# tigert1998/ray-tracing-cuda

Hardware: AMD Instinct MI355X
Metric: Mrays/s (higher is better)
Workload: dtype f32

## Files before the change

ray-tracing-cuda_amd/csrc/capi.hip:

```cpp
#include <hip/hip_runtime.h>
#include <dlfcn.h>
#include <rccl/rccl.h>
#include <string.h>

#include <algorithm>
#include <cmath>
#include <cstdlib>
#include <mutex>
#include <string>
#include <unordered_map>

#include "../../include/rtmi.h"
#include "kernels.h"
#include "scene.h"
#include "xorwow.h"

using namespace rtmi;

static thread_local std::string g_err;
static int fail(int code, const std::string &msg) {
  g_err = msg;
  return code;
}
static int hip_fail(hipError_t e, const char *what) {
  return fail(RTMI_ERR_HIP, std::string(what) + ": " + hipGetErrorString(e));
}
#define HIP_TRY(expr)                                    \
  do {                                                   \
    hipError_t e__ = (expr);                             \
    if (e__ != hipSuccess) return hip_fail(e__, #expr);  \
  } while (0)

// ... 383 lines not shown
  free_device(s);
  std::string err = s->flatten();
  if (!err.empty()) return fail(RTMI_ERR_INVALID, err);
  HIP_TRY(hipGetDevice(&s->device));
  s->tex_recs.clear();
  for (const HostTex &t : s->texs) {
    if (!t.image) continue;
    void *d = nullptr;
    size_t pitch = 0;
    HIP_TRY(hipMallocPitch(&d, &pitch, (size_t)t.w * 4, (size_t)t.h));
    s->dev_allocs.push_back(d);
    HIP_TRY(hipMemcpy2D(d, pitch, t.rgba.data(), (size_t)t.w * 4, (size_t)t.w * 4, (size_t)t.h,
                        hipMemcpyHostToDevice));
    TexRec r{};
    r.rgba = reinterpret_cast<const uint8_t *>(d);
    r.height = t.h, r.width = t.w, r.pitch = (int64_t)pitch;
    s->tex_recs.push_back(r);
  }
  SceneDev d{};
  int rc;
  if ((rc = upload(s, s->runs, &d.runs))) return rc;
  if ((rc = upload(s, s->spheres, &d.spheres))) return rc;
  if ((rc = upload(s, s->tris, &d.tris))) return rc;
  if ((rc = upload(s, s->pair_boxes, &d.pair_boxes))) return rc;
  if ((int)s->pair_pts.size() <= kLdsPairs && (rc = upload(s, s->tri_pts, &d.tri_pts))) return rc;
  if ((rc = upload(s, s->tri_nrm, &d.tri_nrm))) return rc;
  if ((rc = upload(s, s->sph_groups, &d.sph_groups))) return rc;
  if ((rc = upload(s, s->sph_members, &d.sph_members))) return rc;
  d.sph_mag = s->sph_mag;
  d.n_sph_groups = (int)s->sph_groups.size();
  if ((rc = upload(s, s->bvh_recs, &d.bvhs))) return rc;
  if ((rc = upload(s, s->nodes, &d.nodes))) return rc;
  if ((rc = upload(s, s->qnodes, &d.qnodes))) return rc;
  if ((rc = upload(s, s->leaf_paths, &d.leaf_paths))) return rc;
  if ((rc = upload(s, s->tops, &d.tops))) return rc;
  if ((rc = upload(s, s->faces, &d.faces))) return rc;
  if ((rc = upload(s, s->face_uv, &d.face_uv))) return rc;
#ifdef RTMI_CHECK_MARGINS
  if ((rc = upload(s, s->face_of_orig, &d.face_of_orig))) return rc;
#endif
  if ((rc = upload(s, s->mat_recs, &d.mats))) return rc;
  if ((rc = upload(s, s->tex_recs, &d.texs))) return rc;
  d.n_runs = (int)s->runs.size() - 4;
  d.n_pairs = (int)s->pair_pts.size();
  d.list_mag = s->list_mag;
  d.n_mats = (int)s->mat_recs.size();
  d.n_nodes = (int)s->nodes.size();
// ... 59 lines not shown
  Scene tmp;
  if (int rc = flattened(sp, &tmp)) return rc;
  return tmp.sliver_faces;
}

int64_t rtmi_scene_bytes_per_ray(const rtmi_scene *sp) {
  if (!sp) return fail(RTMI_ERR_INVALID, "null scene");
  Scene tmp;
  if (int rc = flattened(sp, &tmp)) return rc;
  return tmp.bytes_per_ray;
}

int64_t rtmi_debug_list_records(const rtmi_scene *sp, int64_t cap_pairs, uint32_t *tri_pts, uint32_t *hot_tris, float *corners) {
  if (!sp) return fail(RTMI_ERR_INVALID, "null scene");
  Scene tmp;
  if (int rc = flattened(sp, &tmp)) return rc;
  const int64_t n = (int64_t)tmp.pair_pts.size();
  for (int64_t i = 0; i < n && i < cap_pairs; i++) {
    if (tri_pts) memcpy(tri_pts + 24 * i, &tmp.tri_pts[2 * i], 2 * sizeof(TriPts));
    if (hot_tris) memcpy(hot_tris + 32 * i, &tmp.tris[2 * i], 2 * sizeof(HotTri));
    if (corners) memcpy(corners + 12 * i, tmp.pair_pts[i].p0, 12 * sizeof(float));
  }
  return n;
}

int64_t rtmi_debug_render_lds_bytes(const rtmi_scene *sp, int max_depth, int threads) {
  if (!sp || max_depth < 0 || threads < 64 || threads % 64) return fail(RTMI_ERR_INVALID, "bad arguments");
  Scene tmp;
  if (int rc = flattened(sp, &tmp)) return rc;
  SceneDev d{};
  d.n_pairs = (int)tmp.pair_pts.size(), d.n_mats = (int)tmp.mat_recs.size(), d.n_nodes = (int)tmp.nodes.size();
  d.n_leaf_paths = (int)tmp.leaf_paths.size(), d.n_sph_groups = (int)tmp.sph_groups.size();
  FrameDev fr{};
  fr.max_depth = max_depth;
  return (int64_t)render_lds_bytes(pick_variant(tmp.features), d, fr, threads);
}

int64_t rtmi_frame_work_items(const rtmi_frame *f) {
  FrameDev d;
  if (!make_frame(f, &d)) return fail(RTMI_ERR_INVALID, frame_why("bad frame"));
  return d.items;
}
int64_t rtmi_frame_pixel_of(const rtmi_frame *f, int64_t q) {
  FrameDev d;
  if (!make_frame(f, &d) || q < 0 || q >= d.items) return -1;
  return frame_pixel_of(d, d.rank, q);
// ... 867 lines not shown
```

ray-tracing-cuda_amd/csrc/closest_hit.h:

```cpp
#pragma once

#ifdef RTMI_CHECK_MARGINS
__device__ inline bool aabb_hit_reference(const BvhNode &nd, V3 o, V3 d, double t_from, double t_to) {
  const float oo[3] = {o.x, o.y, o.z}, dd[3] = {d.x, d.y, d.z};
  for (int i = 0; i < 3; i++) {
    if (dd[i] == 0.f) continue;
    for (int s = 0; s < 2; s++) {
      const float tf = ((s == 0 ? nd.mn[i] : nd.mx[i]) - oo[i]) / dd[i];
      const double t = (double)tf;
      if (t != t || fabs(t) == (double)INFINITY) continue;
      if (!(t_from <= t && t <= t_to)) continue;
      const float pt[3] = {oo[0] + (float)t * dd[0], oo[1] + (float)t * dd[1], oo[2] + (float)t * dd[2]};
      bool inside = true;
      for (int a = 0; a < 3; a++)
        if (a != i && !(nd.mn[a] <= pt[a] && pt[a] <= nd.mx[a])) inside = false;
      if (inside) return true;
    }
  }
  return false;
}
template <typename T>
__device__ inline bool bvh_reference_walk(const SceneDev &sc, const BvhRec &br, V3 o, V3 d, T &t_to, int &face, float &fu,
                                          float &fv) {
  int stk_node[kRefDepthMax + 2], stk_first[kRefDepthMax + 2], stk_n[kRefDepthMax + 2];
// ... 53 lines not shown
                                           , double t_start = INFINITY, double t_stop = INFINITY, bool *uncertain = nullptr
) {
  constexpr bool DT = (F & F_SPHERE) != 0;
  typedef typename TSel<DT>::type T;
  bool ok = false;
  T t_to = OCC ? (T)t_start : (T)INFINITY;
#define RTMI_DECIDED (OCC && ok && t_to <= (T)t_stop)
  uint32_t win = ID_NONE;
  int32_t aux = 0;
  int32_t work = 0;
  float bu = 0.f, bv = 0.f;

  double sa = 0.0, sa2 = 0.0;
  float saf = 0.f;
  if (F & F_SPHERE) {
    float la = len3(d);
    saf = la * la;
    sa = (double)saf;
    sa2 = 2 * sa;
  }

  const int lane = (int)(threadIdx.x & 63u);
  const bool det_safe = (M & PIN_DET_SAFE) || sc.det_safe != 0;
  const bool cull_list = (F & F_TRIS) && ((M & PIN_LDS_TABLES) || (ll != nullptr && sc.n_pairs >= kCullMinPairs));
  V3 cull_inv = splat(0.f), cull_klo = splat(0.f), cull_khi = splat(0.f);
  if ((F & F_TRIS) && cull_list) {
    const float ix = __builtin_amdgcn_rcpf(d.x), iy = __builtin_amdgcn_rcpf(d.y), iz = __builtin_amdgcn_rcpf(d.z);
    cull_inv = mk(fabsf(d.x) < 1e-30f ? copysignf(1e30f, d.x) : ix, fabsf(d.y) < 1e-30f ? copysignf(1e30f, d.y) : iy,
                  fabsf(d.z) < 1e-30f ? copysignf(1e30f, d.z) : iz);
    const float delta = MESH_DIST_SLACK * (fmaxf(fmaxf(fabsf(o.x), fabsf(o.y)), fabsf(o.z)) + sc.list_mag);
    cull_klo = mk(-(o.x + delta) * cull_inv.x, -(o.y + delta) * cull_inv.y, -(o.z + delta) * cull_inv.z);
    cull_khi = mk(-(o.x - delta) * cull_inv.x, -(o.y - delta) * cull_inv.y, -(o.z - delta) * cull_inv.z);
  }

  for (int ri = 0; ri < sc.n_runs; ri++) {
    if (OCC) {
      live = live && !RTMI_DECIDED;
      if (__builtin_amdgcn_ballot_w64(live) == 0ull) break;
    }
    const i32x4 rv = load_run(sc.runs, ri);
    Run run;
    run.kind = rv[0], run.first = rv[1], run.count = rv[2], run.pad = rv[3];
    if (live && run.kind == RUN_SKY) {
      const T ts = (T)1e9f;
      bool hit = ts <= t_to;
      bool acc = hit && (!ok || ts < t_to);
      ok = ok || acc;
      t_to = acc ? ts : t_to;
      win = acc ? make_id(RUN_SKY, 0) : win;
    }
    if ((F & F_TRIS) && run.kind == RUN_TRIS && cull_list) {
      const int pair0 = run.first >> 1;
      const float lo0 = T_FROM_F * kTimeLo;
      for (int c0 = 0; c0 < run.count; c0 += 32) {
        if (OCC && __builtin_amdgcn_ballot_w64(live && !RTMI_DECIDED) == 0ull) break;
        const int nc = run.count - c0 < 32 ? run.count - c0 : 32;
        const float hi0 = (float)t_to * kTimeHi + kTimeAbs;
        uint32_t mask = 0u;
        RTMI_STAT2(const unsigned long long tc0 = stat_now();)
#define RTMI_CULL_PAIR(bx)                                                                                                      \
  {                                                                                                                             \
    const float t0x = __builtin_fmaf(bx[0], cull_inv.x, cull_klo.x), t1x = __builtin_fmaf(bx[3], cull_inv.x, cull_khi.x); \
    const float t0y = __builtin_fmaf(bx[1], cull_inv.y, cull_klo.y), t1y = __builtin_fmaf(bx[4], cull_inv.y, cull_khi.y); \
    const float t0z = __builtin_fmaf(bx[2], cull_inv.z, cull_klo.z), t1z = __builtin_fmaf(bx[5], cull_inv.z, cull_khi.z); \
    const float en = fmaxf(fmaxf(fminf(t0x, t1x), fminf(t0y, t1y)), fminf(t0z, t1z));                                            \
    const float le = fminf(fminf(fmaxf(t0x, t1x), fmaxf(t0y, t1y)), fmaxf(t0z, t1z));                                            \
    cull_step(mask, fmaxf(lo0, en), fminf(hi0, le));                                                                            \
  }
        f32x8 A = load_pair_box(sc.pair_boxes, pair0 + c0), B;
        int i = 0;
        for (; i + 1 < nc; i += 2) {
          __builtin_amdgcn_s_waitcnt(0xc07f);
          __builtin_amdgcn_sched_barrier(0);
          B = load_pair_box(sc.pair_boxes, pair0 + c0 + i + 1);
          __builtin_amdgcn_sched_barrier(0);
          RTMI_CULL_PAIR(A)
          __builtin_amdgcn_s_waitcnt(0xc07f);
          __builtin_amdgcn_sched_barrier(0);
          A = load_pair_box(sc.pair_boxes, pair0 + c0 + i + 2);
          __builtin_amdgcn_sched_barrier(0);
          RTMI_CULL_PAIR(B)
        }
        if (i < nc) {
          __builtin_amdgcn_s_waitcnt(0xc07f);
          __builtin_amdgcn_sched_barrier(0);
          RTMI_CULL_PAIR(A)
        }
#undef RTMI_CULL_PAIR
        mask = __brev(mask) >> (32 - nc);
        if (!live) mask = 0u;
        if (OCC && RTMI_DECIDED) mask = 0u;
        RTMI_STAT2(const unsigned long long tc1 = stat_now(); st.cyc[5] += tc1 - tc0;)
        RTMI_STAT(st.cull_bits += (unsigned)__popcll(__builtin_amdgcn_ballot_w64(true)) * 0u; { unsigned pc = __builtin_popcount(mask); for (int off = 32; off > 0; off >>= 1) pc += __shfl_down(pc, off); st.cull_bits += __builtin_amdgcn_readfirstlane(pc); } st.cull_rays += (unsigned)__popcll(__builtin_amdgcn_ballot_w64(true));)
#ifndef RTMI_OWN_FIRST
#define RTMI_OWN_FIRST 1
#endif
#if RTMI_OWN_FIRST
        if (__builtin_amdgcn_ballot_w64(mask != 0u) != 0ull) {
          if (mask != 0u) {
            const int bit = __builtin_ctz(mask);
            mask &= mask - 1u;
            const int rec = 2 * (pair0 + c0 + bit);
            V3 p0, e1, e2, p1, e1b, e2b;
            (void)load_tri_pts<M>(sc, s_tris, rec, 0, p0, e1, e2);
            const bool second = load_tri_pts<M>(sc, s_tris, rec + 1, 1, p1, e1b, e2b);
            float ta = 0.f, ua = 0.f, va = 0.f, tb = 0.f, ub = 0.f, vb = 0.f;
            const bool hit_a = tri_test_flat<T>(p0, e1, e2, cross3(d, e2), o, d, t_to, ta, ua, va, det_safe);
            bool hit_b = false;
            if (second) hit_b = tri_test_flat<T>(p1, e1b, e2b, cross3(d, e2b), o, d, t_to, tb, ub, vb, det_safe) && !hit_a;
            const float t = hit_a ? ta : tb;
// ... 580 lines not shown
```

ray-tracing-cuda_amd/csrc/kernels.h:

```cpp
#pragma once
#include <hip/hip_runtime.h>
#include <stdint.h>

#include "../../include/rtmi.h"
#include "scene_dev.h"

#define RTMI_KERNEL_MAX_DEPTH 64

namespace rtmi {

int64_t frame_pixel_of(const FrameDev &fr, int rank, int64_t q);

hipError_t launch_rng_init(uint64_t seed, const FrameDev &fr, const uint32_t *d_jump, uint32_t *d_states,
                           hipStream_t stream, int64_t first = -1);

uint32_t pick_variant(uint32_t features);
int render_occupancy(uint32_t variant, const SceneDev &sc, const FrameDev &fr, int threads, bool fast_path = false);
struct RenderTuning {
  int schedule;
  int blocks_per_cu;
  int threads;
  int sparse_stride;
  int exclusive;
  int outlier_x10;
// ... 7 lines not shown
  int prio_every;
  int fast_path;
  int head_classes;
  int first_prio;
  int fetch_batch, fetch_batch_first;
};

enum : uint32_t {
  PIN_NIBBLE_IDS = 1u << 0,
  PIN_LDS_TABLES = 1u << 1,
  PIN_UNSIGNED = 1u << 2,
  PIN_DET_SAFE = 1u << 3,
  PIN_POW2_FRAME = 1u << 4,
  PIN_EVERY_LANE = 1u << 5,
  PIN_PRIORITIES = 1u << 6,
  PIN_CHAINS = 1u << 7,
  PIN_QUEUE = 1u << 8,
};
constexpr uint32_t kFastCommon = PIN_NIBBLE_IDS | PIN_LDS_TABLES | PIN_UNSIGNED | PIN_DET_SAFE | PIN_POW2_FRAME |
                                 PIN_EVERY_LANE | PIN_PRIORITIES;
constexpr uint32_t kFastChains = kFastCommon | PIN_CHAINS;
constexpr uint32_t kFastQueue = kFastCommon | PIN_QUEUE;
constexpr bool defers_unit(uint32_t m) { return (m & kFastCommon) == kFastCommon; }
struct FastPathFacts {
  int enabled;
  uint32_t variant;
  int n_mats;
  int mats_in_lds;
  int pairs_in_lds;
  int unsigned_colours;
  int det_safe;
  int width, height;
  int lane_stride;
  int priorities;
  int chains;
  int resumed;
  int tile_cost;
};
uint32_t fast_path_mode(const FastPathFacts &f);
FastPathFacts fast_path_facts(uint32_t variant, const SceneDev &sc, const FrameDev &fr, int threads, int enabled);
size_t render_lds_bytes(uint32_t variant, const SceneDev &sc, const FrameDev &fr, int threads);
struct SchedPlan {
  const uint32_t *tile_order = nullptr;
  uint32_t *visit_counts = nullptr;
  const uint32_t *sparse_items = nullptr;
  const uint32_t *head_list = nullptr;
  const uint32_t *probe_marks = nullptr;
  int probe_spp = 2;
  uint32_t *prio_tab = nullptr;
  const uint32_t *tile_cost = nullptr;
  const int32_t *chain_next = nullptr;
  const uint32_t *chain_fut = nullptr;
  const int32_t *chain_first = nullptr;
  uint32_t *claims = nullptr;
  int plan_simds = 0, plan_rounds = 0;
};
size_t render_params_bytes();
hipError_t launch_render(uint32_t variant, const SceneDev &sc, const FrameDev &fr, uint32_t *d_states, float *d_out,
                         uint32_t *d_ray_counts, unsigned long long *d_counters, const SchedPlan &plan, bool probe,
                         uint32_t fast, int blocks, int threads, const RenderTuning &tune, void *d_params, hipStream_t stream);
constexpr int kHeadCap = 16384;
hipError_t launch_tile_order(uint32_t *d_ray_counts, int n_tiles, uint32_t *d_cost, uint32_t *d_meta,
                             uint32_t *d_order, uint32_t *d_head, uint32_t sparse_cap, int grid_waves, int outlier_x10,
// ... 66 lines not shown
```

ray-tracing-cuda_amd/csrc/kernels.hip:

```cpp
#include <hip/hip_runtime.h>
#include <stdint.h>

#include "kernels.h"

#include <cstdlib>
#include <iterator>
#include <type_traits>
#include "scene_dev.h"
#include "vec.h"
#include "xorwow.h"

namespace rtmi {

__host__ __device__ __forceinline__ int64_t frame_pixel_of_rank(const FrameDev &fr, int rank, int64_t q) {
  int64_t lt = q >> 6;
  int w = (int)(q & 63);
  int64_t gt = lt * fr.world + rank;
  if (gt >= fr.n_tiles) return -1;
  int ty = (int)(gt / fr.tiles_x), tx = (int)(gt % fr.tiles_x);
  int i = ty * 8 + (w >> 3), j = tx * 8 + (w & 7);
  if (i >= fr.height || j >= fr.width) return -1;
  return (int64_t)i * fr.width + j;
}

int64_t frame_pixel_of(const FrameDev &fr, int rank, int64_t q) { return frame_pixel_of_rank(fr, rank, q); }

__global__ __launch_bounds__(256) void rng_init_kernel(uint64_t seed, FrameDev fr, int64_t first,
// ... 511 lines not shown
    if ((features & ~v) == 0) return v;
  return list[N - 1];
}
uint32_t pick_variant(uint32_t features) { return pick_listed(kVariants, features); }
uint32_t pick_query_variant(uint32_t features) {
  return pick_listed(kQueryVariants, (features & ~(uint32_t)F_DEFOCUS) | F_TEX);
}
template <const auto &List, size_t I = 0, class R, class Fn>
static R with_listed(uint32_t variant, R otherwise, Fn &&f) {
  if constexpr (I == std::size(List)) return otherwise;
  else if (variant == List[I]) return f(std::integral_constant<uint32_t, List[I]>());
  else return with_listed<List, I + 1>(variant, otherwise, f);
}

uint32_t fast_path_mode(const FastPathFacts &f) {
  const auto pow2 = [](int v) { return v > 0 && (v & (v - 1)) == 0 && v <= (1 << 20); };
  const bool common = f.enabled != 0 && f.variant == (uint32_t)F_TRIS && f.n_mats >= 1 && f.n_mats <= 16 && f.mats_in_lds != 0 &&
                      f.pairs_in_lds != 0 && f.unsigned_colours != 0 && f.det_safe != 0 && pow2(f.width) && pow2(f.height) &&
                      f.lane_stride == 1 && f.priorities != 0;
  if (!common) return 0u;
  if (!f.chains) return kFastQueue;
  return f.resumed && f.tile_cost ? kFastChains : 0u;
}
FastPathFacts fast_path_facts(uint32_t variant, const SceneDev &sc, const FrameDev &fr, int threads, int enabled) {
  size_t lds = 0;
  const LaunchCfg lc = make_cfg(variant, sc, fr, threads, &lds);
  FastPathFacts f{};
  f.enabled = enabled, f.variant = variant, f.n_mats = sc.n_mats, f.mats_in_lds = lc.lds_mats > 0 && lc.wide_ids == 2;
  f.pairs_in_lds = lc.pairs_off >= 0 && lc.nrm_off >= 0 && lc.list_off >= 0;
  f.unsigned_colours = sc.unsigned_colours, f.det_safe = sc.det_safe, f.width = fr.width, f.height = fr.height;
  return f;
}

size_t render_lds_bytes(uint32_t variant, const SceneDev &sc, const FrameDev &fr, int threads) {
  size_t lds = 0;
  (void)make_cfg(variant, sc, fr, threads, &lds);
  return lds;
}

template <auto Kernel>
static hipError_t kernel_occupancy(int threads, size_t lds, int *per_cu) {
  *per_cu = 0;
  if (lds > 160 * 1024) return hipErrorInvalidConfiguration;
  hipError_t e = dynamic_lds<Kernel>(lds);
  if (e == hipSuccess) e = hipOccupancyMaxActiveBlocksPerMultiprocessor(per_cu, Kernel, threads, lds);
  if (e != hipSuccess) *per_cu = 0;
  return e;
}
struct LaunchAt {
  int blocks, threads;
  size_t lds;
  hipStream_t stream;
// ... 49 lines not shown
    lc.promote = tune.promote;
    lc.lane_stride = tune.lane_stride > 0 ? tune.lane_stride : 1;
    lc.prio_tab = plan.prio_tab;
    lc.tile_cost = plan.tile_cost;
    lc.rate_scale = 1.f / (64.f * (float)(plan.probe_spp > 0 ? plan.probe_spp : 1));
    lc.chain_next = (F & F_BVH) || lc.prio_tab == nullptr ? nullptr : plan.chain_next;
    lc.chain_fut = plan.chain_fut, lc.chain_first = plan.chain_first, lc.claims = plan.claims;
    lc.plan_simds = plan.plan_simds, lc.plan_rounds = plan.plan_rounds;
    lc.prio_every = tune.prio_every > 0 ? tune.prio_every : 16;
    {
      const int samples = fr.k_end - fr.k_begin > 0 ? fr.k_end - fr.k_begin : 1;
      const int by_length = 4096 / samples < 1 ? 1 : 4096 / samples;
      lc.fetch_batch = probe && samples <= 4 ? tune.fetch_batch_first : plan.tile_order != nullptr ? std::min(by_length, tune.fetch_batch) : image_order_batch(samples, 16);
    }
    RenderParams rp;
    rp.sc = sc, rp.fr = fr, rp.lc = lc;
    rp.states = d_states, rp.out = d_out, rp.ray_counts = d_ray_counts, rp.counters = d_counters;
    RenderParams *dp = reinterpret_cast<RenderParams *>(d_params);
    const LaunchAt at{blocks, threads, lds, stream};
    if constexpr (F == (uint32_t)F_TRIS) {
      const bool chains = fast == kFastChains && !probe && lc.chain_next && lc.tile_cost && fr.k_begin > 0 && d_ray_counts;
      const bool queue = fast == kFastQueue && !lc.chain_next;
      if (fast != 0u && (!lc.prio_tab || lc.lane_stride != 1 || !(chains || queue))) return hipErrorInvalidValue;
      if (chains) return launch_block<render_kernel<F, kFastChains>>(at, rp, dp);
      if (queue && !probe) return launch_block<render_kernel<F, kFastQueue>>(at, rp, dp);
      if (queue) return launch_block<probe_kernel<F, kFastQueue>>(at, rp, dp);
    }
    if (fast != 0u) return hipErrorInvalidValue;
    if (probe) return launch_block<probe_kernel<F>>(at, rp, dp);
    return launch_block<render_kernel<F>>(at, rp, dp);
  });
}

hipError_t launch_untile(const FrameDev &fr, const float *d_tiles, float *d_image, hipStream_t stream) {
  int64_t total = fr.items * fr.world;
  if (total == 0) return hipSuccess;
  hipLaunchKernelGGL((untile_kernel<float, 3>), dim3((unsigned)cdiv(total, 256)), dim3(256), 0, stream, fr, d_tiles,
                     d_image);
  return hipGetLastError();
}

hipError_t launch_untile_u32(const FrameDev &fr, const uint32_t *d_tiles, uint32_t *d_image, hipStream_t stream) {
  int64_t total = fr.items * fr.world;
  if (total == 0) return hipSuccess;
  hipLaunchKernelGGL((untile_kernel<uint32_t, 1>), dim3((unsigned)cdiv(total, 256)), dim3(256), 0, stream, fr,
                     d_tiles, d_image);
// ... 272 lines not shown
```

ray-tracing-cuda_amd/csrc/margins.h:

```cpp
#pragma once

namespace rtmi {

constexpr float kEps32 = 0x1p-24f;
constexpr float kReachMeasured = 2.1f;
constexpr float kReachProvided = 8.0f;
constexpr float kThinSine = 1.0f / 32.0f;
constexpr float kDistSlack = 0x1p-16f;
constexpr float kPadOfExtent = 1e-4f;
constexpr float kPadOfMagnitude = 1e-5f;
constexpr float kPadFloor = 1e-30f;
constexpr float kTimeLo = 0.999f, kTimeHi = 1.0001f, kTimeAbs = 1e-6f;
constexpr float kSlabTimeRel = 1e-5f;
constexpr float kSphReach = 7.75e-4f;
constexpr float kSphDiscRel = 1e-5f;
constexpr float kSphDistSlack = 0x1p-9f;
constexpr float kSphRadiusPad = 0x1p-10f;
constexpr float kSqrt3 = 1.7320508f;

static_assert(kDistSlack >= kReachProvided * kEps32 / kThinSine, "the distance slack must provide 8 eps / sin(theta) down to the thin-face limit");
static_assert(kReachProvided >= kReachMeasured * kSqrt3, "the provision must cover the measured reach with D taken in the max norm");
static_assert(kPadOfExtent >= kReachMeasured * kEps32 / kThinSine * 4.0f, "the fixed pad covers the reach at distances of the bounds' own size");
static_assert(kPadOfMagnitude >= 8.0f * kEps32, "the fixed pad covers the rounding of the slab arithmetic (a reciprocal and an FMA per plane)");
static_assert(kSphDistSlack >= kSphReach * kSqrt3, "the sphere groups' slack must cover the binary32 pre-test's reach");
static_assert(kTimeLo < 1.0f - 64.0f * kEps32 && kTimeHi > 1.0f + 64.0f * kEps32 && kSlabTimeRel > 64.0f * kEps32,
              "the time fudges must be far above the few-eps disagreement of two operation orders");

inline float fixed_pad(float diag, float mag) { return kPadOfExtent * diag + kPadOfMagnitude * mag + kPadFloor; }

}
```

ray-tracing-cuda_amd/csrc/scene.h:

```cpp
#pragma once
#include <stdint.h>

#include <string>
#include <vector>

#include "scene_dev.h"
#include "vec.h"

namespace rtmi {

struct HostTex {
  bool image = false;
  V3 rgb{0, 0, 0};
  std::vector<uint8_t> rgba;
  int h = 0, w = 0;
};

struct HostMat {
  int32_t kind = MAT_LAMBERTIAN;
  V3 rgb{0, 0, 0};
  float param = 0.f;
  int tex = -1;
};

// ... 13 lines not shown
  int n = 0, mat = -1, leaf_max = 2048;
};

struct PairPts {
  float p0[3], p1[3], p2[3], p3[3];
};

struct Scene {
  std::vector<HostTex> texs;
  std::vector<HostMat> mats;
  std::vector<HostObj> world;
  std::vector<int> list_counts{0};
  std::vector<HostBvh> bvhs;
  CameraDev cam{};
  V3 cam_w{0, 0, 0};
  bool has_camera = false;

  bool committed = false;
  uint32_t features = 0;
  std::vector<Run> runs;
  std::vector<SphereRec> spheres;
  std::vector<HotTri> tris;
  std::vector<PairBox> pair_boxes;
  std::vector<PairPts> pair_pts;
  std::vector<TriPts> tri_pts;
  std::vector<TriNrm> tri_nrm;
  std::vector<SphGroup> sph_groups;
  std::vector<SphMember> sph_members;
  float sph_mag = 0.f;
  int64_t sliver_faces = 0;
  float list_mag = 0.f;
  int n_pgrams = 0, n_triangles = 0, n_spheres = 0;
  std::vector<BvhRec> bvh_recs;
  std::vector<BvhNode> nodes;
  std::vector<QNode4> qnodes;
  std::vector<BvhNode> tops;
  std::vector<int32_t> leaf_paths;
  int sub_depth = 0;
  std::vector<FaceRec> faces;
  std::vector<float> face_uv;
  std::vector<int32_t> face_of_orig;
  std::vector<MatRec> mat_recs;
  std::vector<TexRec> tex_recs;
  std::vector<int32_t> q_sphere_entry, q_pair_entry, q_bvh_entry, q_face_input;
  int32_t q_sky_entry = -1;
  std::vector<void *> dev_allocs;
// ... 21 lines not shown
```

ray-tracing-cuda_amd/csrc/scene.hip:

```cpp
#include "scene.h"

#include <algorithm>
#include <cmath>
#include <cstring>
#include <numeric>

namespace rtmi {

TriRec make_tri(V3 p0, V3 p1, V3 p2) {
  V3 e1 = p1 - p0, e2 = p2 - p0;
  V3 n = unit3(cross3(e1, e2));
  TriRec r;
  r.p0[0] = p0.x, r.p0[1] = p0.y, r.p0[2] = p0.z;
  r.e1[0] = e1.x, r.e1[1] = e1.y, r.e1[2] = e1.z;
  r.e2[0] = e2.x, r.e2[1] = e2.y, r.e2[2] = e2.z;
  r.n[0] = n.x, r.n[1] = n.y, r.n[2] = n.z;
  return r;
}

static HotTri hot_tri(V3 p0, V3 p1, V3 p2, int mat, int flags) {
  TriRec t = make_tri(p0, p1, p2);
  HotTri h{};
  for (int c = 0; c < 3; c++) h.p0[c] = t.p0[c], h.e1[c] = t.e1[c], h.e2[c] = t.e2[c], h.n[c] = t.n[c];
  h.mat = mat;
// ... 26 lines not shown
  const V3 q[4] = {p[0], p[1], p[2], n == 4 ? p[3] : p[2]};
  for (int c = 0; c < 3; c++) {
    const float x[4] = {c == 0 ? q[0].x : c == 1 ? q[0].y : q[0].z, c == 0 ? q[1].x : c == 1 ? q[1].y : q[1].z,
                        c == 0 ? q[2].x : c == 1 ? q[2].y : q[2].z, c == 0 ? q[3].x : c == 1 ? q[3].y : q[3].z};
    pp.p0[c] = x[0], pp.p1[c] = x[1], pp.p2[c] = x[2], pp.p3[c] = x[3];
  }
  PairBox bx{};
  float diag = 0.f, mag = 0.f;
  for (int c = 0; c < 3; c++) {
    const float x[4] = {pp.p0[c], pp.p1[c], pp.p2[c], pp.p3[c]};
    bx.mn[c] = fminf(fminf(x[0], x[1]), fminf(x[2], x[3]));
    bx.mx[c] = fmaxf(fmaxf(x[0], x[1]), fmaxf(x[2], x[3]));
    diag = fmaxf(diag, bx.mx[c] - bx.mn[c]);
    mag = fmaxf(mag, fmaxf(fabsf(bx.mn[c]), fabsf(bx.mx[c])));
  }
  const float pad = fixed_pad(diag, mag);
  for (int c = 0; c < 3; c++) bx.mn[c] -= pad, bx.mx[c] += pad;
  const V3 second[3] = {q[1], q[2], q[3]};
  if (face_slack_exponent(q) > 0 || (n == 4 && face_slack_exponent(second) > 0))
    for (int c = 0; c < 3; c++) bx.mn[c] = -INFINITY, bx.mx[c] = INFINITY;
  s.list_mag = fmaxf(s.list_mag, mag);
  s.pair_pts.push_back(pp);
  s.pair_boxes.push_back(bx);
}

static void push_pgram(Scene &s, V3 p0, V3 p1, V3 p2, int mat) {
  std::vector<HotTri> &out = s.tris;
  V3 p3 = p1 + p2 - p0;
  const HotTri first = hot_tri(p0, p1, p2, mat, TRI_PGRAM);
  HotTri second = hot_tri(p1, p2, p3, mat, TRI_PGRAM | TRI_SECOND);
  if (memcmp(first.e2, second.e2, sizeof(first.e2)) == 0) second.flags |= TRI_SAME_E2;
  out.push_back(first);
  out.push_back(second);
  const V3 q[4] = {p0, p1, p2, p3};
  push_pair(s, q, 4);
}

void box_from_points(const V3 p[4], V3 out[8]) {
  auto fourth = [](V3 a, V3 b, V3 c) { return c + b - a; };
  V3 q[4];
  q[3] = fourth(p[0], p[1], p[2]);
  q[2] = fourth(p[0], p[1], p[3]);
  q[1] = fourth(p[0], p[2], p[3]);
  q[0] = fourth(p[1], q[2], q[3]);
  for (int i = 0; i < 4; i++) out[i] = p[i], out[4 + i] = q[i];
}
// ... 393 lines not shown
    }
  int me = (int)nodes.size();
  nodes.push_back(nd);
  if (level > 0) path.push_back(me);
  if (n <= leaf_max) {
    nodes[me].left = -1;
    nodes[me].right = -n;
    for (int i = 0; i < n; i++) fp[first + i].code = code, fp[first + i].leaf = (int)leaf_paths.size();
    leaf_paths.push_back(path);
  } else {
    int mid = (n - 1) / 2;
    const uint32_t bit = level < 32 ? 0x80000000u >> level : 0u;
    int l = build_bvh_nodes(nodes, fp, first, mid + 1, leaf_max, level + 1, code, ref_depth, path, leaf_paths);
    int r = build_bvh_nodes(nodes, fp, first + mid + 1, n - mid - 1, leaf_max, level + 1, code | bit, ref_depth, path,
                            leaf_paths);
    nodes[me].left = l;
    nodes[me].right = r;
  }
  if (level > 0) path.pop_back();
  return me;
}

std::string Scene::flatten() {
  pair_boxes.clear(), pair_pts.clear(), tri_pts.clear(), tri_nrm.clear(), list_mag = 0.f;
  sph_groups.clear(), sph_members.clear(), sph_mag = 0.f;
  sliver_faces = 0;
  runs.clear(), spheres.clear(), tris.clear(), bvh_recs.clear(), face_of_orig.clear(), nodes.clear(), qnodes.clear(), faces.clear(), leaf_paths.clear(), tops.clear(),
      face_uv.clear(), mat_recs.clear(), tex_recs.clear();
  q_sphere_entry.clear(), q_pair_entry.clear(), q_bvh_entry.clear(), q_face_input.clear(), q_sky_entry = -1;
  features = 0;
  n_pgrams = n_triangles = n_spheres = 0;
  sub_depth = 0;
  if (!has_camera) return "scene has no camera";
  if (list_counts.empty() || list_counts[0] > 1024) return "world exceeds HitableList::kMaxHitables (1024)";
  if (cam.defocus) features |= F_DEFOCUS;

  std::vector<int> tex_to_image(texs.size(), -1);
  int n_images = 0;
  for (size_t i = 0; i < texs.size(); i++)
    if (texs[i].image) tex_to_image[i] = n_images++;
  for (const HostMat &m : mats) {
    MatRec r{};
    r.kind = m.kind;
    r.r = m.rgb.x, r.g = m.rgb.y, r.b = m.rgb.z;
    r.param = m.param;
    r.tex = -1;
    if (m.tex >= 0) {
// ... 241 lines not shown
      float diag = 0.f, mag = 0.f;
      for (int a = 0; a < 3; a++) diag = fmaxf(diag, mx[a] - mn[a]), mag = fmaxf(mag, fmaxf(fabsf(mn[a]), fabsf(mx[a])));
      const float pad = fixed_pad(diag, mag) + kSphDistSlack * mag;
      for (int a = 0; a < 3; a++) g.mn[a] = mn[a] - pad, g.mx[a] = mx[a] + pad;
      sph_mag = fmaxf(sph_mag, mag);
      sph_groups.push_back(g);
    }
  }
  if (!sph_groups.empty()) features |= F_SGROUP;
  if (!sph_groups.empty()) {
    sph_groups.push_back(SphGroup{});
    sph_members.push_back(SphMember{});
  }
  for (size_t t = 0; t < 2 * pair_pts.size() && t < tris.size(); t++) {
    TriNrm r{};
    for (int c = 0; c < 3; c++) r.n[c] = tris[t].n[c];
    r.mat_flags = (tris[t].mat & 0xffffff) | (tris[t].flags << 24);
    tri_nrm.push_back(r);
  }
  if (!tris.empty()) {
    tris.push_back(HotTri{});
    tris.push_back(HotTri{});
    pair_boxes.push_back(PairBox{});
  }
  n_spheres = (int)spheres.size();
  if (!spheres.empty()) spheres.push_back(SphereRec{});
  for (const MatRec &m : mat_recs)
    if (m.tex >= 0) bytes_per_ray += 4;
  return check_margins();
}

std::string Scene::check_margins() const {
  for (size_t i = 0; i < pair_pts.size(); i++) {
    const PairPts &pp = pair_pts[i];
    const PairBox &bx = pair_boxes[i];
    const bool lone = !(tris[2 * i].flags & TRI_PGRAM);
    const V3 q[4] = {mk(pp.p0[0], pp.p0[1], pp.p0[2]), mk(pp.p1[0], pp.p1[1], pp.p1[2]), mk(pp.p2[0], pp.p2[1], pp.p2[2]),
                     lone ? mk(pp.p2[0], pp.p2[1], pp.p2[2]) : mk(pp.p3[0], pp.p3[1], pp.p3[2])};
    const V3 second[3] = {q[1], q[2], q[3]};
    const bool thin = face_slack_exponent(q) > 0 || (!lone && face_slack_exponent(second) > 0);
    float mn[3] = {INFINITY, INFINITY, INFINITY}, mx[3] = {-INFINITY, -INFINITY, -INFINITY};
    for (int j = 0; j < 4; j++) {
      const float c[3] = {q[j].x, q[j].y, q[j].z};
      for (int a = 0; a < 3; a++) mn[a] = fminf(mn[a], c[a]), mx[a] = fmaxf(mx[a], c[a]);
    }
    float diag = 0.f, mag = 0.f;
    for (int a = 0; a < 3; a++) diag = fmaxf(diag, mx[a] - mn[a]), mag = fmaxf(mag, fmaxf(fabsf(mn[a]), fabsf(mx[a])));
    const double pad = 0.98 * (double)fixed_pad(diag, mag);
    for (int a = 0; a < 3; a++) {
      if (thin ? !(bx.mn[a] == -INFINITY && bx.mx[a] == INFINITY)
               : !((double)bx.mn[a] <= (double)mn[a] - pad && (double)bx.mx[a] >= (double)mx[a] + pad))
        return "margin budget: a world-list pair's bounds do not cover what its triangle tests can accept";
    }
    if (!(mag <= list_mag)) return "margin budget: list_mag is below a pair's coordinates";
  }
  if (tri_pts.size() != 2 * pair_pts.size() || tris.size() < tri_pts.size()) return "world list: triangle records out of step";
  for (size_t t = 0; t < tri_pts.size(); t++) {
    const bool absent = (t & 1) && !(tris[t].flags & TRI_SECOND);
    if (absent != ((tri_pts[t].flags & TRIPTS_ABSENT) != 0)) return "world list: a triangle record's absent flag is wrong";
    if (!absent && memcmp(tri_pts[t].p0, tris[t].p0, 9 * sizeof(float)) != 0)
      return "world list: a triangle record's base point or edges differ from its HotTri's";
  }
  for (size_t g = 0; g + 1 < sph_groups.size(); g++) {
    const SphGroup &gr = sph_groups[g];
    float mn[3] = {INFINITY, INFINITY, INFINITY}, mx[3] = {-INFINITY, -INFINITY, -INFINITY};
    for (int k = 0; k < gr.count; k++) {
      const SphMember &m = sph_members[(size_t)gr.first + k];
      const double r = std::fabs(spheres[(size_t)m.orig].radius) * (1.0 + (double)kSphRadiusPad) * 0.999999;
      const float c[3] = {m.cx, m.cy, m.cz};
      for (int a = 0; a < 3; a++) mn[a] = fminf(mn[a], (float)((double)c[a] - r)), mx[a] = fmaxf(mx[a], (float)((double)c[a] + r));
    }
    float diag = 0.f, mag = 0.f;
    for (int a = 0; a < 3; a++) diag = fmaxf(diag, mx[a] - mn[a]), mag = fmaxf(mag, fmaxf(fabsf(mn[a]), fabsf(mx[a])));
    const double pad = 0.98 * ((double)fixed_pad(diag, mag) + (double)kSphDistSlack * mag);
    for (int a = 0; a < 3; a++)
      if (!((double)gr.mn[a] <= (double)mn[a] - pad && (double)gr.mx[a] >= (double)mx[a] + pad))
        return "margin budget: a sphere group's bounds do not cover what its members' pre-tests can accept";
// ... 28 lines not shown
```

ray-tracing-cuda_amd/csrc/scene_dev.h:

```cpp
#pragma once
#include <stdint.h>

#include "vec.h"
#include "margins.h"

namespace rtmi {

enum RunKind : int32_t { RUN_SKY = 0, RUN_SPHERE = 1, RUN_TRIS = 2, RUN_BVH = 4 };

struct Run {
  int32_t kind, first, count, pad;
};

struct SphereRec {
  float cx, cy, cz;
  int32_t mat;
  double radius;
  double r2;
};

struct SphGroup {
  float mn[3], mx[3];
  int32_t first, count;
};
// ... 11 lines not shown
struct TriRec {
  float p0[3];
  float e1[3];
  float e2[3];
  float n[3];
};

enum : int32_t { TRI_SECOND = 1, TRI_PGRAM = 2, TRI_SAME_E2 = 4 };
struct HotTri {
  float p0[3];
  float e1[3];
  float e2[3];
  float n[3];
  int32_t mat;
  int32_t flags;
  int32_t pad[2];
};

enum : int32_t { TRIPTS_ABSENT = 1 };
struct PairBox {
  float mn[3], mx[3];
  int32_t pad[2];
};
struct alignas(16) TriPts {
  float p0[3], e1[3], e2[3];
  int32_t flags;
  int32_t pad[2];
};
static_assert(sizeof(TriPts) == 48, "TriPts is read with three ds_read_b128");
struct alignas(16) TriNrm {
  float n[3];
  int32_t mat_flags;
};
constexpr int kMaxStackMats = 1 << 16;
constexpr int kMaxMats = 1 << 24;
constexpr int kCullMinPairs = 4;
constexpr int kListTasks(uint32_t features) { return (features & 16u) ? 96 : (features & 4u) ? 128 : 192; }
constexpr int kListWaveWords(uint32_t features) {
  return 64 * 8 + kListTasks(features) * (1 + ((features & 16u) ? 6 : (features & 1u) ? 3 : 2));
}
constexpr int kLdsPairs = 128;

enum MatKind : int32_t { MAT_LAMBERTIAN = 0, MAT_METAL = 1, MAT_DIELECTRIC = 2, MAT_LIGHT = 3, MAT_SKY = 4 };

struct alignas(16) MatRec {
  float r, g, b;
// ... 154 lines not shown
```

ray-tracing-cuda_amd/rtmi/__init__.py:

```python
import collections
import ctypes as C
import os

import numpy as np

_PKG_DIR = os.path.dirname(os.path.abspath(__file__))
_ROOT = os.path.dirname(_PKG_DIR)
LIB_PATH = os.environ.get("RTMI_LIB_PATH") or os.path.join(_ROOT, "lib", "librtmi.so")

TILE = 8
STATE_WORDS = 6
MAX_DEPTH = 64
TRACE_WORK_WORDS = 256
BUDGET_WORK_WORDS = TRACE_WORK_WORDS
MODE_FIELDS = 9
FAST_PATH_FACTS = 14
MAX_MATERIALS = 1 << 24

RTMI_HIT_NONE = 0
RTMI_HIT_SPHERE = 1
RTMI_HIT_TRIANGLE = 2
RTMI_HIT_PARALLELOGRAM = 3
RTMI_HIT_PARALLELEPIPED = 4
RTMI_HIT_MESH = 5
# ... 521 lines not shown
        finally:
            self.L.rtmi_scene_destroy(tmp)
        return self.camera_update(f)

    def random_float(self, mn, mx):
        return np.float32(self.L.rtmi_rng_host_random_float(C.c_float(float(np.float32(mn))),
                                                            C.c_float(float(np.float32(mx))),
                                                            self.state0.ctypes.data_as(_u32p)))

    def stats(self):
        out = (C.c_int64 * 8)()
        _check(self.L.rtmi_scene_stats(self.h, out), "rtmi_scene_stats")
        keys = ["world", "spheres", "parallelograms", "triangles", "bvh_faces", "bvh_nodes", "materials", "textures"]
        return dict(zip(keys, list(out)))

    def list_records(self):
        fn = self.L.rtmi_debug_list_records
        fn.restype, fn.argtypes = C.c_int64, [C.c_void_p, C.c_int64, _u32p, _u32p, _fp]
        n = _check(fn(self.h, 0, None, None, None), "rtmi_debug_list_records")
        tp, ht, co = np.zeros((n, 2, 12), np.uint32), np.zeros((n, 2, 16), np.uint32), np.zeros((n, 4, 3), np.float32)
        _check(fn(self.h, n, tp.ctypes.data_as(_u32p), ht.ctypes.data_as(_u32p), co.ctypes.data_as(_fp)), "rtmi_debug_list_records")
        return tp, ht, co

    def render_lds_bytes(self, max_depth, threads=256):
        fn = self.L.rtmi_debug_render_lds_bytes
        fn.restype, fn.argtypes = C.c_int64, [C.c_void_p, C.c_int, C.c_int]
        return _check(fn(self.h, max_depth, threads), "rtmi_debug_render_lds_bytes")

    def sliver_faces(self):
        return _check(self.L.rtmi_scene_sliver_faces(self.h), "rtmi_scene_sliver_faces")

    def bytes_per_ray(self):
        return _check(self.L.rtmi_scene_bytes_per_ray(self.h), "rtmi_scene_bytes_per_ray")

    def commit(self):
        _check(self.L.rtmi_scene_commit(self.h), "rtmi_scene_commit")
        self.device = None
        try:
            import torch
            if torch.cuda.is_available():
                self.device = torch.device("cuda", torch.cuda.current_device())
        except ImportError:
            pass
        return self

    def intersect(self, origins, directions, t_max=None, out=None):
# ... 341 lines not shown
```

Before: 33910.

## Precompute widened center/half-extent slab table for world-list pair culling

Adds a second table of per-pair slab records (center and half-extent, pre-widened on the host by the distance slack plus rounding margin for origins within a fixed reach) uploaded after the pair boxes. The fast-path kernels read this table and cull with fewer per-ray setup ops and FMA-based slab tests, dropping the per-ray delta widening. A host check gates the fast path on the camera lying within the reach, and the margin validator verifies coverage. This costs extra device memory and conservatively wider boxes, which may let more pairs through the cull.

```diff
diff --git a/ray-tracing-cuda_amd/csrc/capi.hip b/ray-tracing-cuda_amd/csrc/capi.hip
--- a/ray-tracing-cuda_amd/csrc/capi.hip
+++ b/ray-tracing-cuda_amd/csrc/capi.hip
@@ -8,6 +8,7 @@
 #include <cstdlib>
 #include <mutex>
 #include <string>
+#include <type_traits>
 #include <unordered_map>
 
 #include "../../include/rtmi.h"
@@ -437,7 +438,13 @@
   if ((rc = upload(s, s->runs, &d.runs))) return rc;
   if ((rc = upload(s, s->spheres, &d.spheres))) return rc;
   if ((rc = upload(s, s->tris, &d.tris))) return rc;
-  if ((rc = upload(s, s->pair_boxes, &d.pair_boxes))) return rc;
+  {
+    static_assert(sizeof(PairSlab) == sizeof(PairBox) && std::is_trivially_copyable<PairSlab>::value, "PairSlab records travel as PairBox");
+    std::vector<PairBox> both(s->pair_boxes);
+    both.resize(s->pair_boxes.size() + s->pair_slabs.size());
+    if (!s->pair_slabs.empty()) memcpy(both.data() + s->pair_boxes.size(), s->pair_slabs.data(), s->pair_slabs.size() * sizeof(PairSlab));
+    if ((rc = upload(s, both, &d.pair_boxes))) return rc;
+  }
   if ((int)s->pair_pts.size() <= kLdsPairs && (rc = upload(s, s->tri_pts, &d.tri_pts))) return rc;
   if ((rc = upload(s, s->tri_nrm, &d.tri_nrm))) return rc;
   if ((rc = upload(s, s->sph_groups, &d.sph_groups))) return rc;
@@ -543,6 +550,26 @@
     if (corners) memcpy(corners + 12 * i, tmp.pair_pts[i].p0, 12 * sizeof(float));
   }
   return n;
+}
+
+int64_t rtmi_debug_pair_slabs(const rtmi_scene *sp, int64_t cap, uint32_t *slabs, uint32_t *boxes, float *list_mag) {
+  if (!sp) return fail(RTMI_ERR_INVALID, "null scene");
+  Scene tmp;
+  if (int rc = flattened(sp, &tmp)) return rc;
+  const int64_t n = (int64_t)tmp.pair_slabs.size();
+  for (int64_t i = 0; i < n && i < cap; i++) {
+    if (slabs) memcpy(slabs + 8 * i, &tmp.pair_slabs[i], sizeof(PairSlab));
+    if (boxes) memcpy(boxes + 8 * i, &tmp.pair_boxes[i], sizeof(PairBox));
+  }
+  if (list_mag) *list_mag = tmp.list_mag;
+  return n;
+}
+
+int rtmi_debug_slab_reach(const rtmi_scene *sp) {
+  if (!sp) return fail(RTMI_ERR_INVALID, "null scene");
+  Scene tmp;
+  if (int rc = flattened(sp, &tmp)) return rc;
+  return slab_reach_covers(tmp.list_mag, tmp.cam) ? 1 : 0;
 }
 
 int64_t rtmi_debug_render_lds_bytes(const rtmi_scene *sp, int max_depth, int threads) {
diff --git a/ray-tracing-cuda_amd/csrc/closest_hit.h b/ray-tracing-cuda_amd/csrc/closest_hit.h
--- a/ray-tracing-cuda_amd/csrc/closest_hit.h
+++ b/ray-tracing-cuda_amd/csrc/closest_hit.h
@@ -99,15 +99,20 @@
 
   const int lane = (int)(threadIdx.x & 63u);
   const bool det_safe = (M & PIN_DET_SAFE) || sc.det_safe != 0;
+  constexpr bool SLAB = culls_by_slab(M);
   const bool cull_list = (F & F_TRIS) && ((M & PIN_LDS_TABLES) || (ll != nullptr && sc.n_pairs >= kCullMinPairs));
   V3 cull_inv = splat(0.f), cull_klo = splat(0.f), cull_khi = splat(0.f);
   if ((F & F_TRIS) && cull_list) {
     const float ix = __builtin_amdgcn_rcpf(d.x), iy = __builtin_amdgcn_rcpf(d.y), iz = __builtin_amdgcn_rcpf(d.z);
     cull_inv = mk(fabsf(d.x) < 1e-30f ? copysignf(1e30f, d.x) : ix, fabsf(d.y) < 1e-30f ? copysignf(1e30f, d.y) : iy,
                   fabsf(d.z) < 1e-30f ? copysignf(1e30f, d.z) : iz);
-    const float delta = MESH_DIST_SLACK * (fmaxf(fmaxf(fabsf(o.x), fabsf(o.y)), fabsf(o.z)) + sc.list_mag);
-    cull_klo = mk(-(o.x + delta) * cull_inv.x, -(o.y + delta) * cull_inv.y, -(o.z + delta) * cull_inv.z);
-    cull_khi = mk(-(o.x - delta) * cull_inv.x, -(o.y - delta) * cull_inv.y, -(o.z - delta) * cull_inv.z);
+    if (SLAB) {
+      cull_klo = mk(-o.x * cull_inv.x, -o.y * cull_inv.y, -o.z * cull_inv.z);
+    } else {
+      const float delta = MESH_DIST_SLACK * (fmaxf(fmaxf(fabsf(o.x), fabsf(o.y)), fabsf(o.z)) + sc.list_mag);
+      cull_klo = mk(-(o.x + delta) * cull_inv.x, -(o.y + delta) * cull_inv.y, -(o.z + delta) * cull_inv.z);
+      cull_khi = mk(-(o.x - delta) * cull_inv.x, -(o.y - delta) * cull_inv.y, -(o.z - delta) * cull_inv.z);
+    }
   }
 
   for (int ri = 0; ri < sc.n_runs; ri++) {
@@ -144,25 +149,40 @@
     const float le = fminf(fminf(fmaxf(t0x, t1x), fmaxf(t0y, t1y)), fmaxf(t0z, t1z));                                            \
     cull_step(mask, fmaxf(lo0, en), fminf(hi0, le));                                                                            \
   }
-        f32x8 A = load_pair_box(sc.pair_boxes, pair0 + c0), B;
+#define RTMI_CULL_SLAB(bx)                                                                                                      \
+  {                                                                                                                             \
+    const float tcx = __builtin_fmaf(bx[0], cull_inv.x, cull_klo.x), tcy = __builtin_fmaf(bx[1], cull_inv.y, cull_klo.y),       \
+                tcz = __builtin_fmaf(bx[2], cull_inv.z, cull_klo.z);                                                            \
+    const float nx = __builtin_fmaf(-bx[3], fabsf(cull_inv.x), tcx), fx = __builtin_fmaf(bx[3], fabsf(cull_inv.x), tcx);        \
+    const float ny = __builtin_fmaf(-bx[4], fabsf(cull_inv.y), tcy), fy = __builtin_fmaf(bx[4], fabsf(cull_inv.y), tcy);        \
+    const float nz = __builtin_fmaf(-bx[5], fabsf(cull_inv.z), tcz), fz = __builtin_fmaf(bx[5], fabsf(cull_inv.z), tcz);        \
+    const float en = fmaxf(fmaxf(nx, ny), nz), le = fminf(fminf(fx, fy), fz);                                                   \
+    cull_step_nlt(mask, fminf(hi0, le), fmaxf(lo0, en));                                                                        \
+  }
+#define RTMI_CULL_ONE(bx)  \
+  if (SLAB) RTMI_CULL_SLAB(bx) else RTMI_CULL_PAIR(bx)
+        const PairBox *const recs = sc.pair_boxes;
+        f32x8 A = load_pair_box(recs, pair0 + c0), B;
         int i = 0;
         for (; i + 1 < nc; i += 2) {
           __builtin_amdgcn_s_waitcnt(0xc07f);
           __builtin_amdgcn_sched_barrier(0);
-          B = load_pair_box(sc.pair_boxes, pair0 + c0 + i + 1);
+          B = load_pair_box(recs, pair0 + c0 + i + 1);
           __builtin_amdgcn_sched_barrier(0);
-          RTMI_CULL_PAIR(A)
+          RTMI_CULL_ONE(A)
           __builtin_amdgcn_s_waitcnt(0xc07f);
           __builtin_amdgcn_sched_barrier(0);
-          A = load_pair_box(sc.pair_boxes, pair0 + c0 + i + 2);
+          A = load_pair_box(recs, pair0 + c0 + i + 2);
           __builtin_amdgcn_sched_barrier(0);
-          RTMI_CULL_PAIR(B)
+          RTMI_CULL_ONE(B)
         }
         if (i < nc) {
           __builtin_amdgcn_s_waitcnt(0xc07f);
           __builtin_amdgcn_sched_barrier(0);
-          RTMI_CULL_PAIR(A)
-        }
+          RTMI_CULL_ONE(A)
+        }
+#undef RTMI_CULL_ONE
+#undef RTMI_CULL_SLAB
 #undef RTMI_CULL_PAIR
         mask = __brev(mask) >> (32 - nc);
         if (!live) mask = 0u;
diff --git a/ray-tracing-cuda_amd/csrc/kernels.h b/ray-tracing-cuda_amd/csrc/kernels.h
--- a/ray-tracing-cuda_amd/csrc/kernels.h
+++ b/ray-tracing-cuda_amd/csrc/kernels.h
@@ -53,6 +53,7 @@
 constexpr uint32_t kFastChains = kFastCommon | PIN_CHAINS;
 constexpr uint32_t kFastQueue = kFastCommon | PIN_QUEUE;
 constexpr bool defers_unit(uint32_t m) { return (m & kFastCommon) == kFastCommon; }
+constexpr bool culls_by_slab(uint32_t m) { return (m & kFastCommon) == kFastCommon; }
 struct FastPathFacts {
   int enabled;
   uint32_t variant;
@@ -70,6 +71,7 @@
 };
 uint32_t fast_path_mode(const FastPathFacts &f);
 FastPathFacts fast_path_facts(uint32_t variant, const SceneDev &sc, const FrameDev &fr, int threads, int enabled);
+bool slab_reach_covers(float list_mag, const CameraDev &cam);
 size_t render_lds_bytes(uint32_t variant, const SceneDev &sc, const FrameDev &fr, int threads);
 struct SchedPlan {
   const uint32_t *tile_order = nullptr;
diff --git a/ray-tracing-cuda_amd/csrc/kernels.hip b/ray-tracing-cuda_amd/csrc/kernels.hip
--- a/ray-tracing-cuda_amd/csrc/kernels.hip
+++ b/ray-tracing-cuda_amd/csrc/kernels.hip
@@ -3,6 +3,8 @@
 
 #include "kernels.h"
 
+#include <cfloat>
+#include <cmath>
 #include <cstdlib>
 #include <iterator>
 #include <type_traits>
@@ -560,12 +562,18 @@
   if (!f.chains) return kFastQueue;
   return f.resumed && f.tile_cost ? kFastChains : 0u;
 }
+bool slab_reach_covers(float list_mag, const CameraDev &cam) {
+  const float reach = kOriginReach * list_mag;
+  const bool cam_in_reach = fabsf(cam.position.x) <= reach && fabsf(cam.position.y) <= reach && fabsf(cam.position.z) <= reach;
+  const bool k_finite = (double)(kOriginReach + 1.0f) * (double)list_mag * 1e30 < (double)FLT_MAX;
+  return cam_in_reach && k_finite;
+}
 FastPathFacts fast_path_facts(uint32_t variant, const SceneDev &sc, const FrameDev &fr, int threads, int enabled) {
   size_t lds = 0;
   const LaunchCfg lc = make_cfg(variant, sc, fr, threads, &lds);
   FastPathFacts f{};
   f.enabled = enabled, f.variant = variant, f.n_mats = sc.n_mats, f.mats_in_lds = lc.lds_mats > 0 && lc.wide_ids == 2;
-  f.pairs_in_lds = lc.pairs_off >= 0 && lc.nrm_off >= 0 && lc.list_off >= 0;
+  f.pairs_in_lds = lc.pairs_off >= 0 && lc.nrm_off >= 0 && lc.list_off >= 0 && slab_reach_covers(sc.list_mag, sc.cam);
   f.unsigned_colours = sc.unsigned_colours, f.det_safe = sc.det_safe, f.width = fr.width, f.height = fr.height;
   return f;
 }
@@ -661,6 +669,8 @@
       const bool chains = fast == kFastChains && !probe && lc.chain_next && lc.tile_cost && fr.k_begin > 0 && d_ray_counts;
       const bool queue = fast == kFastQueue && !lc.chain_next;
       if (fast != 0u && (!lc.prio_tab || lc.lane_stride != 1 || !(chains || queue))) return hipErrorInvalidValue;
+      static_assert(culls_by_slab(kFastChains) && culls_by_slab(kFastQueue) && !culls_by_slab(0u), "which kernels read the slab table");
+      if (chains || queue) rp.sc.pair_boxes = pair_slabs_of(sc.pair_boxes, sc.n_pairs);
       if (chains) return launch_block<render_kernel<F, kFastChains>>(at, rp, dp);
       if (queue && !probe) return launch_block<render_kernel<F, kFastQueue>>(at, rp, dp);
       if (queue) return launch_block<probe_kernel<F, kFastQueue>>(at, rp, dp);
diff --git a/ray-tracing-cuda_amd/csrc/margins.h b/ray-tracing-cuda_amd/csrc/margins.h
--- a/ray-tracing-cuda_amd/csrc/margins.h
+++ b/ray-tracing-cuda_amd/csrc/margins.h
@@ -17,15 +17,24 @@
 constexpr float kSphDistSlack = 0x1p-9f;
 constexpr float kSphRadiusPad = 0x1p-10f;
 constexpr float kSqrt3 = 1.7320508f;
+constexpr float kOriginReach = 8.0f;
+constexpr float kSlabRoundEps = 8.0f;
 
 static_assert(kDistSlack >= kReachProvided * kEps32 / kThinSine, "the distance slack must provide 8 eps / sin(theta) down to the thin-face limit");
 static_assert(kReachProvided >= kReachMeasured * kSqrt3, "the provision must cover the measured reach with D taken in the max norm");
 static_assert(kPadOfExtent >= kReachMeasured * kEps32 / kThinSine * 4.0f, "the fixed pad covers the reach at distances of the bounds' own size");
 static_assert(kPadOfMagnitude >= 8.0f * kEps32, "the fixed pad covers the rounding of the slab arithmetic (a reciprocal and an FMA per plane)");
+static_assert(kSlabRoundEps * (kOriginReach + 1.0f) >= 5.0f * (kOriginReach + 2.01f),
+              "the slab table's rounding term covers three roundings and the reciprocal's 2 eps of (|o| + |c| + h') at an origin kOriginReach mag out");
+static_assert(kOriginReach >= 1.0f, "origins on the list's own triangles must be within the slab table's reach");
 static_assert(kSphDistSlack >= kSphReach * kSqrt3, "the sphere groups' slack must cover the binary32 pre-test's reach");
 static_assert(kTimeLo < 1.0f - 64.0f * kEps32 && kTimeHi > 1.0f + 64.0f * kEps32 && kSlabTimeRel > 64.0f * kEps32,
               "the time fudges must be far above the few-eps disagreement of two operation orders");
 
 inline float fixed_pad(float diag, float mag) { return kPadOfExtent * diag + kPadOfMagnitude * mag + kPadFloor; }
 
+inline double slab_widening(float list_mag) {
+  return ((double)kDistSlack + (double)kSlabRoundEps * (double)kEps32) * ((double)kOriginReach + 1.0) * (double)list_mag;
 }
+
+}
diff --git a/ray-tracing-cuda_amd/csrc/scene.h b/ray-tracing-cuda_amd/csrc/scene.h
--- a/ray-tracing-cuda_amd/csrc/scene.h
+++ b/ray-tracing-cuda_amd/csrc/scene.h
@@ -59,6 +59,7 @@
   std::vector<SphereRec> spheres;
   std::vector<HotTri> tris;
   std::vector<PairBox> pair_boxes;
+  std::vector<PairSlab> pair_slabs;
   std::vector<PairPts> pair_pts;
   std::vector<TriPts> tri_pts;
   std::vector<TriNrm> tri_nrm;
diff --git a/ray-tracing-cuda_amd/csrc/scene.hip b/ray-tracing-cuda_amd/csrc/scene.hip
--- a/ray-tracing-cuda_amd/csrc/scene.hip
+++ b/ray-tracing-cuda_amd/csrc/scene.hip
@@ -72,6 +72,24 @@
   s.list_mag = fmaxf(s.list_mag, mag);
   s.pair_pts.push_back(pp);
   s.pair_boxes.push_back(bx);
+}
+
+static PairSlab pair_slab(const PairBox &bx, float list_mag) {
+  PairSlab r{};
+  const double widen = slab_widening(list_mag);
+  for (int a = 0; a < 3; a++) {
+    const double lo = (double)bx.mn[a] - widen, hi = (double)bx.mx[a] + widen;
+    const float c = (float)((lo + hi) / 2);
+    const double h = std::fmax(hi - (double)c, (double)c - lo);
+    float hf = (float)h;
+    if ((double)hf < h) hf = nextafterf(hf, INFINITY);
+    r.c[a] = c, r.h[a] = hf;
+  }
+  bool bounded = true;
+  for (int a = 0; a < 3; a++) bounded = bounded && std::isfinite(r.c[a]) && std::isfinite(r.h[a]);
+  if (!bounded)
+    for (int a = 0; a < 3; a++) r.c[a] = 0.f, r.h[a] = INFINITY;
+  return r;
 }
 
 static void push_pgram(Scene &s, V3 p0, V3 p1, V3 p2, int mat) {
@@ -511,7 +529,7 @@
 }
 
 std::string Scene::flatten() {
-  pair_boxes.clear(), pair_pts.clear(), tri_pts.clear(), tri_nrm.clear(), list_mag = 0.f;
+  pair_boxes.clear(), pair_slabs.clear(), pair_pts.clear(), tri_pts.clear(), tri_nrm.clear(), list_mag = 0.f;
   sph_groups.clear(), sph_members.clear(), sph_mag = 0.f;
   sliver_faces = 0;
   runs.clear(), spheres.clear(), tris.clear(), bvh_recs.clear(), face_of_orig.clear(), nodes.clear(), qnodes.clear(), faces.clear(), leaf_paths.clear(), tops.clear(),
@@ -799,6 +817,8 @@
     tris.push_back(HotTri{});
     tris.push_back(HotTri{});
     pair_boxes.push_back(PairBox{});
+    for (size_t i = 0; i + 1 < pair_boxes.size(); i++) pair_slabs.push_back(pair_slab(pair_boxes[i], list_mag));
+    pair_slabs.push_back(PairSlab{});
   }
   n_spheres = (int)spheres.size();
   if (!spheres.empty()) spheres.push_back(SphereRec{});
@@ -830,6 +850,15 @@
         return "margin budget: a world-list pair's bounds do not cover what its triangle tests can accept";
     }
     if (!(mag <= list_mag)) return "margin budget: list_mag is below a pair's coordinates";
+    if (pair_slabs.size() != pair_boxes.size()) return "margin budget: the slab table is out of step with the pair bounds";
+    const PairSlab &sl = pair_slabs[i];
+    const double widen = slab_widening(list_mag) * (1.0 - 0x1p-40);
+    for (int a = 0; a < 3; a++) {
+      if (thin ? !(sl.c[a] == 0.f && sl.h[a] == INFINITY)
+               : !(((double)sl.c[a] - (double)sl.h[a] <= (double)bx.mn[a] - widen && (double)sl.c[a] + (double)sl.h[a] >= (double)bx.mx[a] + widen) ||
+                   (sl.c[a] == 0.f && sl.h[a] == INFINITY)))
+        return "margin budget: a world-list pair's slab record does not cover its bounds at the edge of the origin reach";
+    }
   }
   if (tri_pts.size() != 2 * pair_pts.size() || tris.size() < tri_pts.size()) return "world list: triangle records out of step";
   for (size_t t = 0; t < tri_pts.size(); t++) {
diff --git a/ray-tracing-cuda_amd/csrc/scene_dev.h b/ray-tracing-cuda_amd/csrc/scene_dev.h
--- a/ray-tracing-cuda_amd/csrc/scene_dev.h
+++ b/ray-tracing-cuda_amd/csrc/scene_dev.h
@@ -57,6 +57,12 @@
   float mn[3], mx[3];
   int32_t pad[2];
 };
+struct PairSlab {
+  float c[3], h[3];
+  int32_t pad[2];
+};
+static_assert(sizeof(PairSlab) == sizeof(PairBox), "the slab table is addressed in PairBox records");
+inline const PairBox *pair_slabs_of(const PairBox *boxes, int32_t n_pairs) { return boxes + n_pairs + 1; }
 struct alignas(16) TriPts {
   float p0[3], e1[3], e2[3];
   int32_t flags;
diff --git a/ray-tracing-cuda_amd/rtmi/__init__.py b/ray-tracing-cuda_amd/rtmi/__init__.py
--- a/ray-tracing-cuda_amd/rtmi/__init__.py
+++ b/ray-tracing-cuda_amd/rtmi/__init__.py
@@ -567,6 +567,19 @@
         _check(fn(self.h, n, tp.ctypes.data_as(_u32p), ht.ctypes.data_as(_u32p), co.ctypes.data_as(_fp)), "rtmi_debug_list_records")
         return tp, ht, co
 
+    def pair_slabs(self):
+        fn = self.L.rtmi_debug_pair_slabs
+        fn.restype, fn.argtypes = C.c_int64, [C.c_void_p, C.c_int64, _u32p, _u32p, _fp]
+        n = _check(fn(self.h, 0, None, None, None), "rtmi_debug_pair_slabs")
+        sl, bx, mag = np.zeros((n, 8), np.uint32), np.zeros((n, 8), np.uint32), np.zeros(1, np.float32)
+        _check(fn(self.h, n, sl.ctypes.data_as(_u32p), bx.ctypes.data_as(_u32p), mag.ctypes.data_as(_fp)), "rtmi_debug_pair_slabs")
+        return sl.view(np.float32), bx.view(np.float32), float(mag[0])
+
+    def slab_reach(self):
+        fn = self.L.rtmi_debug_slab_reach
+        fn.restype, fn.argtypes = C.c_int, [C.c_void_p]
+        return bool(_check(fn(self.h), "rtmi_debug_slab_reach"))
+
     def render_lds_bytes(self, max_depth, threads=256):
         fn = self.L.rtmi_debug_render_lds_bytes
         fn.restype, fn.argtypes = C.c_int64, [C.c_void_p, C.c_int, C.c_int]
```

After: 35670 (median of 6 runs). 1.05x the previous value.
